# mojing1999/jmcodec

Measured on AMD Instinct MI355X. Metric: decoded frames/sec @1080p H.264 + bit-exact YUV, higher is better.
Workload: dtype u8

## Files before the change

### jmcodec_amd/csrc/decoder.cpp

```cpp
#include "decoder.h"
#include "numa.h"
#include <pthread.h>
#include <time.h>
#include "engine.h"
#include "host_copy.h"
#include "kernels.h"
#include <hip/hip_runtime_api.h>
#include <algorithm>
#include <cstdio>
#include <cstdlib>
#include <cstring>
#include <thread>

namespace jmamd {

#define HIP_OK(expr) ((expr) == hipSuccess)

namespace {
int thread_budget() {
    const char *e = getenv("JM_AMD_DEC_THREADS");
    int n = e ? atoi(e) : (int)std::thread::hardware_concurrency();
    if (!e) {
        if (FILE *f = fopen("/sys/fs/cgroup/cpu.max", "r")) {
            long long q = 0, per = 0; char qs[32] = {0};
// ... 129 lines not shown
    if (k == "field_pictures") return stat_field_pics_.load();
    if (k == "lone_fields") return stat_lone_fields_.load();
    if (k == "frames") return num_frames_;
    if (k == "out_width") return out_w_;
    if (k == "out_height") return out_h_;
    if (k == "scaled_frames") return stat_scaled_;
    if (k == "rgb_frames") return stat_rgb_;
    if (k == "deint_frames") return stat_deint_;
    if (k == "field_rate_pairs") return stat_pairs_;
    if (k == "interlaced_sequence") return codec_ == 0 && seq_active_ && !seq_.frame_mbs_only ? 1 : 0;
    if (k == "out_frame_bytes") { std::lock_guard<std::mutex> lk(const_cast<std::mutex &>(mtx_));
        return (long long)(cur_out_ ? cur_out_->fbytes : !ready_.empty() ? ready_.front()->fbytes : frame_bytes_); }
    if (k == "out_slot_bytes") { std::lock_guard<std::mutex> lk(const_cast<std::mutex &>(mtx_)); long long n = 0;
        for (const OutSlot *o : all_out_) n += (o->host ? (long long)o->bytes : 0) + (o->dev ? (long long)o->bytes : 0); return n; }
    if (k == "vui_full_range") return vui_[0];
    if (k == "vui_primaries") return vui_[1];
    if (k == "vui_transfer") return vui_[2];
    if (k == "vui_matrix") return vui_[3];
    if (k == "color_matrix") return color_matrix_;
    if (k == "color_range") return color_range_;
    if (k == "pictures") return stat_pictures_;
    if (k == "job_bytes") return stat_job_bytes_;
    if (k == "job_regrown") return stat_job_regrown_;
    if (k == "job_slot_bytes") { long long n = 0; for (auto &j : jobs_) n += (long long)j.cap; return n; }
    if (k == "errors") return stat_errors_;
    if (k == "jpeg_pictures") return stat_jpeg_pics_;
    if (k == "jpeg_sampling") return codec_ == 2 && seq_active_ ? j_sampling_ : 0;
    if (k == "jpeg_restart_intervals") return stat_jpeg_ri_;
    if (k == "copy_engines") return copier_ ? (long long)copier_->engine_mask() : 0;
    if (k == "direct_frames") return stat_direct_;
    if (k == "direct_ns") return stat_direct_ns_;
    if (k == "device_wait_errors") return stat_wait_errors_;
    if (k == "intra_mbs") return stat_intra_mbs_;
    if (k == "coef_int16") return stat_coef_;
    if (k == "syntax_digest") return codec_ == 1 ? (long long)hdigest_.h : (long long)digest_.h;
    if (k == "job_digest") return (long long)job_digest_;
    if (k == "digest_mbs") return codec_ == 1 ? (long long)hdigest_.n_cu : (long long)digest_.mbs;
    if (k == "i_pictures") return stat_i_;
    if (k == "p_pictures") return stat_p_;
    if (k == "b_pictures") return stat_b_;
    if (k == "fps_num") return codec_ == 1 ? (long long)hsps_.time_scale : (long long)seq_.time_scale;
    if (k == "fps_den") return codec_ == 1 ? (long long)hsps_.num_units_in_tick : 2ll * seq_.num_units_in_tick;
    if (k == "out_fps_num") { const bool chosen = deint_when_ == 1 || (codec_ == 0 && seq_active_ && !seq_.frame_mbs_only);
        return (field_rate() && chosen ? 2 : 1) * get_stat("fps_num"); }
    if (k == "out_fps_den") return get_stat("fps_den");
    if (k == "frames_done_unfetched") return (long long)frames_done_unfetched();
    if (k == "frames_waiting") { std::lock_guard<std::mutex> lk(const_cast<std::mutex &>(mtx_)); return (long long)ready_.size(); }
    if (k == "pictures_in_flight") { std::lock_guard<std::mutex> lk(const_cast<std::mutex &>(mtx_)); return (long long)outstanding_; }
    if (k == "coded_width") return mb_w_ * 16;
    if (k == "coded_height") return mb_h_ * 16;
    if (k == "pitch") return pitch_;
    if (k == "device") return device_;
    if (k == "threads") return pool_threads(numa_node_);
    if (k == "numa_node") return numa_node_;
    if (k == "elapsed_us") return (long long)(elapsed_ms_ * 1000.0);
    if (k == "parse_ns_i") return stat_parse_ns_i_;
    if (k == "submit_ns") return stat_submit_ns_;
    if (k == "wait_slot_ns") return stat_wait_slot_ns_;
    if (k == "parse_ns_p") return stat_parse_ns_p_;
    if (k.rfind("k_", 0) == 0 || k.rfind("eng_", 0) == 0) {
        static const char *kn[kKernelClasses] = {"inter", "intra", "deblock", "packout", "chain", "rgb_pack", "deint", "jpeg"};
        if (!engine_) return 0;
        EngineStats es = engine_->stats();
        for (int i = 0; i < kKernelClasses; i++) {
            if (k == std::string("k_") + kn[i] + "_ns") return (long long)es.ns[i];
            if (k == std::string("k_") + kn[i] + "_n") return es.launches[i];
// ... 1073 lines not shown
    mv_ext_buf.resize((size_t)n_mbs * (big_rec ? kBiRecInt16 : 32));
    const size_t fixed = (size_t)n_mbs * sizeof(MbRec) + 256 * sizeof(SliceRec);
    MbRec *mbs = nullptr; SliceRec *srec = nullptr; int16_t *coef = nullptr;
    MbRec blank; memset(&blank, 0, sizeof blank); blank.kind = MB_INTER;
    { int8_t c = -1; for (auto &s : t->slices) if (s.sh.type != SL_I && s.refs.slot[0][0] >= 0) { c = s.refs.slot[0][0]; break; }
      blank.ref[0] = blank.ref[1] = blank.ref[2] = blank.ref[3] = c; }
    JobWriter w;
    SyntaxDigest dg = digest_;
    for (int attempt = 0;; attempt++) {
        scratch.begin_picture();
        mbs = (MbRec *)js.host; srec = (SliceRec *)(js.host + (size_t)n_mbs * sizeof(MbRec)); coef = (int16_t *)(srec + 256);
        w = JobWriter();
        w.mbs = mbs; w.mv_ext = mv_ext_buf.data(); w.mv_ext_cap = (uint32_t)n_mbs * (big_rec ? kBiRecInt16 / 2 : 16);
        w.coef = coef;
        {
            long long room = (long long)js.cap - (long long)fixed - 64;
            if (room <= 0) { t->error = "job buffer too small for this picture"; stat_errors_++; fail(t->error); room = 0; }
            w.coef_cap = (uint32_t)(room / 2);
        }
        dg = digest_;
        t->n_intra = 0; t->n_i8x8 = 0; t->any_deblock = false; t->any_wp = false; t->error.clear();
        const char *first_error = nullptr; bool overflow = false;
        for (size_t si = 0; si < t->slices.size(); si++) {
            SliceTask &s = t->slices[si];
            srec[si].alpha_off = (int8_t)s.sh.alpha_off; srec[si].beta_off = (int8_t)s.sh.beta_off; srec[si].disable = (uint8_t)s.sh.disable_deblock;
            srec[si].pad = 0;
            if (s.sh.disable_deblock != 1) t->any_deblock = true;
            BitReader br(s.rbsp.data(), s.rbsp_len);
            br.set_end_from_trailing();
            br.skip_bytes(s.sh.data_bit_offset >> 3); br.skip((int)(s.sh.data_bit_offset & 7));
            if (s.sh.first_mb >= n_mbs) { t->error = "first_mb_in_slice out of range"; continue; }
            if (s.col) s.col->wait();
            if (s.has_wp) t->any_wp = true;
            SliceParseResult r = parse_slice_data(t->sps, t->pps, s.sh, br, (int)si, s.refs, scratch, w, want_digest_ ? &dg : nullptr, fast_parse_ &&
                !t->field);
            t->n_intra += r.n_intra; t->n_i8x8 += r.n_i8x8;
            if (r.error) { t->error = r.error; if (!first_error) first_error = r.error; overflow |= strcmp(r.error, "coefficient buffer overflow") == 0; }
        }
        if (overflow && js.cap < job_cap_max_ && attempt < 6 && !failed_) {
            const bool i_pic = !t->slices.empty() && t->slices[0].sh.type == SL_I;
            const size_t want = std::min(job_cap_max_, std::max(js.cap * 2, i_pic ? i_job_peak_.load() * 5 / 4 : (size_t)0));
            if (ensure_job_cap(js, want)) { stat_job_regrown_++; continue; }
        }
        if (!t->error.empty()) { stat_errors_++; note_error(std::string("slice data: ") + t->error); }
        break;
    }
    for (int i = 0; i < n_mbs; i++) if (scratch.slice_of[i] < 0) mbs[i] = blank;
    if (want_digest_) digest_ = dg;
    if (const char *dm = getenv("JM_AMD_DEC_DUMP_MB")) {
        int dp = 0, dx = 0, dy = 0;
        if (sscanf(dm, "%d:%d:%d", &dp, &dx, &dy) == 3 && (dp < 0 || dp == (int)stat_pictures_.load())) {
            for (int oy = -1; oy <= 0; oy++) for (int ox = -1; ox <= 1; ox++) {
                const int x = dx + ox, y = dy + oy;
                if (x < 0 || y < 0 || x >= t->sps.mb_w || y >= t->sps.mb_h || (oy == 0 && ox == 1)) continue;
                const MbRec &m = mbs[y * t->sps.mb_w + x];
                fprintf(stderr, "MB(%d,%d) kind %d flags 0x%02x modes 0x%02x qp %d slice %d cbp_blk 0x%04x i4 %02x%02x%02x%02x%02x%02x%02x%02x "
                        "n_intra %d n_i8x8 %d slice_type %d\n", x, y, m.kind, m.flags, m.modes, m.qp, m.slice, m.cbp_blk,
                        m.u.i4[0], m.u.i4[1], m.u.i4[2], m.u.i4[3], m.u.i4[4], m.u.i4[5], m.u.i4[6], m.u.i4[7], t->n_intra, t->n_i8x8,
                            t->slices.empty() ? -1 : (int)t->slices[0].sh.type);
            }
        }
    }
    t->n_slices = (int)t->slices.size();
    if (t->mf) {
        MotionField &f = *t->mf;
        size_t n = (size_t)n_mbs;
        f.mv[0].assign(scratch.mv.begin(), scratch.mv.begin() + n * 32); f.mv[1].assign(scratch.mv1.begin(), scratch.mv1.begin() + n * 32);
        f.ref[0].assign(scratch.refidx.begin(), scratch.refidx.begin() + n * 4); f.ref[1].assign(scratch.refidx1.begin(), scratch.refidx1.begin() + n * 4);
        f.uid[0].assign(scratch.uid0.begin(), scratch.uid0.begin() + n * 4); f.uid[1].assign(scratch.uid1.begin(), scratch.uid1.begin() + n * 4);
// ... 359 lines not shown
```

### jmcodec_amd/csrc/decoder.h

```cpp
#pragma once
#include "h264_cavlc.h"
#include "h264_syntax.h"
#include "hevc_slice.h"
#include "jpeg_syntax.h"
#include "jobs.h"
#include "scale_packed.h"
#include <atomic>
#include <chrono>
#include <condition_variable>
#include <deque>
#include <memory>
#include <mutex>
#include <string>
#include <vector>

struct ihipStream_t; struct ihipEvent_t;

namespace jmamd {

constexpr int kMaxJobSlots = 64;
constexpr int kJobSlots = 24;
constexpr int kJobSlotsSmall = 40;
constexpr int kJpegJobSlots = 16, kJpegSurfaces = 18;

// ... 224 lines not shown
    std::deque<std::unique_ptr<PicTask>> inflight_;
    std::mutex submit_mtx_;
    JobSlot jobs_[kMaxJobSlots]; int n_jobs_ = kJobSlots;
    bool n_jobs_set_ = false;
    BigJobBuf big_[kBigJobBufs];
    void free_job_buffers();
    std::deque<OutSlot *> ready_;
    std::atomic<int> done_unfetched_{0};
    std::vector<OutSlot *> free_out_, all_out_;
    OutSlot *cur_out_ = nullptr;
    int outstanding_ = 0, parse_pending_ = 0;

    struct EngineDecoderState *eng_state_ = nullptr;
    class Engine *engine_ = nullptr;
    uint8_t *surf_[kMaxSurfaces] = {nullptr};
    uint8_t *surf_block_ = nullptr;
    void free_surfaces();
    bool use_lds_deblock_ = false;
    uint8_t *resid_ = nullptr; bool use_lds_intra_ = false; bool lds_intra8_ = false;
    uint8_t *hevc_work_[kHevcWorkSets] = {nullptr, nullptr, nullptr, nullptr}; unsigned hevc_work_rr_ = 0;
    uint8_t *hevc_bs_ = nullptr; size_t hevc_bs_set_bytes_ = 0, hevc_bs_off_[4] = {0, 0, 0, 0};
    int pitch_ = 0, chroma_off_ = 0; size_t surf_bytes_ = 0, frame_bytes_ = 0, job_cap_ = 0, job_cap_max_ = 0;
    std::atomic<size_t> i_job_peak_{0};
    std::atomic<long long> stat_job_regrown_{0};
    bool gpu_open_ = false;

    bool eof_flag_ = false, is_exit_ = false;
    std::atomic<bool> eos_sent_{false};
    uint32_t num_frames_ = 0;
    std::chrono::steady_clock::time_point t0_; bool timer_started_ = false; double elapsed_ms_ = 0;
    char info_[1024];
    std::atomic<long long> stat_parse_ns_i_{0}, stat_parse_ns_p_{0}, stat_submit_ns_{0}, stat_wait_slot_ns_{0};
    std::atomic<long long> stat_pictures_{0}, stat_job_bytes_{0}, stat_errors_{0}, stat_intra_mbs_{0}, stat_coef_{0}, stat_wait_errors_{0};
    SyntaxDigest digest_;
    bool fast_parse_ = true, want_job_digest_ = false;
    std::atomic<long long> stat_direct_{0}, stat_direct_ns_{0};
    HostCopier *copier_ = nullptr; uint64_t out_sig_ = 0;
    int display_delay_ = 0;
    uint64_t job_digest_ = 1469598103934665603ull;
    HevcParamSets hps_; HevcSps hsps_; HevcPps hpps_;
    int h_poc_tid0_ = 0, h_max_dpb_ = 1, h_reorder_ = 0, extra_surf_ = 0; bool h_first_picture_ = true, h_no_rasl_output_ = false, h_seen_eos_ = false;
    HevcSliceHeader h_last_sh_; bool h_have_last_sh_ = false;
    HevcDigest hdigest_;
    long long stat_i_ = 0, stat_p_ = 0, stat_b_ = 0;
    std::vector<int> display_pocs_;
    std::vector<uint8_t> display_fields_;
    std::vector<uint32_t> display_pics_;
    uint32_t display_count_ = 0;
    JpegSplitter jsplit_; JpegTables jtab_;
    int j_w_ = 0, j_h_ = 0, j_sampling_ = 0; unsigned j_surf_rr_ = 0;
    std::atomic<long long> stat_jpeg_pics_{0}, stat_jpeg_ri_{0};
    struct TraceRec { uint64_t seq; long long t_dispatch, t_parsed, t_submit0, t_submit1; int is_i; };
    std::vector<TraceRec> trace_; bool trace_on_ = false;
};

void pool_submit(Decoder *d, PicTask *t);
int  pool_threads(int numa_node);

}
```

### jmcodec_amd/csrc/h264_cavlc.cpp

```cpp
#include "h264_cavlc.h"
#include "h264_cabac.h"
#include <mutex>
#include <stddef.h>
#include <emmintrin.h>

namespace jmamd {

static const uint8_t kTokLen[3][68] = {
{ 1,0,0,0, 6,2,0,0, 8,6,3,0, 9,8,7,5, 10,9,8,6, 11,10,9,7, 13,11,10,8, 13,13,11,9, 13,13,13,10,
 14,14,13,11, 14,14,14,13, 15,15,14,14, 15,15,15,14, 16,15,15,15, 16,16,16,15, 16,16,16,16, 16,16,16,16 },
{ 2,0,0,0, 6,2,0,0, 6,5,3,0, 7,6,6,4, 8,6,6,4, 8,7,7,5, 9,8,8,6, 11,9,9,6, 11,11,11,7,
 12,11,11,9, 12,12,12,11, 12,12,12,11, 13,13,13,12, 13,13,13,13, 13,14,13,13, 14,14,14,13, 14,14,14,14 },
{ 4,0,0,0, 6,4,0,0, 6,5,4,0, 6,5,5,4, 7,5,5,4, 7,5,5,4, 7,6,6,4, 7,6,6,4, 8,7,7,5,
 8,8,7,6, 9,8,8,7, 9,9,8,8, 9,9,9,8, 10,9,9,9, 10,10,10,10, 10,10,10,10, 10,10,10,10 } };
static const uint8_t kTokBits[3][68] = {
{ 1,0,0,0, 5,1,0,0, 7,4,1,0, 7,6,5,3, 7,6,5,3, 7,6,5,4, 15,6,5,4, 11,14,5,4, 8,10,13,4,
 15,14,9,4, 11,10,13,12, 15,14,9,12, 11,10,13,8, 15,1,9,12, 11,14,13,8, 7,10,9,12, 4,6,5,8 },
{ 3,0,0,0, 11,2,0,0, 7,7,3,0, 7,10,9,5, 7,6,5,4, 4,6,5,6, 7,6,5,8, 15,6,5,4, 11,14,13,4,
 15,10,9,4, 11,14,13,12, 8,10,9,8, 15,14,13,12, 11,10,9,12, 7,11,6,8, 9,8,10,1, 7,6,5,4 },
{ 15,0,0,0, 15,14,0,0, 11,15,13,0, 8,12,14,12, 15,10,11,11, 11,8,9,10, 9,14,13,9, 8,10,9,8, 15,14,13,13,
 11,14,10,12, 15,10,13,12, 11,14,9,12, 8,10,13,8, 13,7,9,12, 9,12,11,10, 5,8,7,6, 1,4,3,2 } };
static const uint8_t kCdcLen[20] = { 2,0,0,0, 6,1,0,0, 6,6,3,0, 6,7,7,6, 6,8,8,7 };
static const uint8_t kCdcBits[20] = { 1,0,0,0, 7,1,0,0, 4,6,1,0, 3,3,2,5, 2,3,2,0 };
static const uint8_t kTzLen[15][16] = {
// ... 91 lines not shown
    mb_w = w; mb_h = h;
    size_t n = (size_t)w * h;
    tc.assign(n * 24, 0); mv.assign(n * 32, 0); refidx.assign(n * 4, -1); i4.assign(n * 16, 2); info.assign(n, 0); slice_of.assign(n, -1);
    cbp.assign(n, 0); cmode.assign(n, 0); cbf.assign(n, 0); mvd.assign(n * 32, 0);
    mv1.assign(n * 32, 0); refidx1.assign(n * 4, -1); mvd1.assign(n * 32, 0); direct8.assign(n, 0); uid0.assign(n * 4, -1); uid1.assign(n * 4, -1);
}
void ParseScratch::begin_picture() { std::fill(slice_of.begin(), slice_of.end(), (int16_t)-1); }

namespace {

struct Canon {
    uint32_t addr; uint8_t kind , qp, cmode, i16mode; uint8_t i4[16]; int8_t ref[4];
    int16_t mv[16][2];
    int16_t i16dc[16], luma[16][16], cdc[2][4], cac[2][4][16];
    int8_t ref1[4]; int16_t mv1[16][2];
};
static_assert(sizeof(Canon) == 4 + 4 + 16 + 4 + 64 + 32 + 512 + 16 + 256 + 4 + 64, "Canon must be packed");

struct P {
    const SeqParams &sps; const PicParamSet &pps; const SliceHeader &sh;
    BitReader &br; ParseScratch &cx; JobWriter &out; SyntaxDigest *dg;
    int slice_num; const SliceRefs &rf;
    int mb_w, mb_x = 0, mb_y = 0, addr = 0, qp;
    int nA = -1, nB = -1, nC = -1, nD = -1;
    uint8_t *tc; int16_t *mv; int8_t *ref; uint8_t *i4m;
    int16_t *mvl[2]; int8_t *refl[2]; uint8_t *mvdl[2];
    uint32_t decoded_mask = 0;
    Canon *canon = nullptr;
    Cabac *cb = nullptr;
    const uint8_t *zz4 = kZigzag4, *zz8 = kZigzag8; int fld_ctx = 0;
    bool last_dqp = false;
    uint8_t *mvd = nullptr;
    const char *err = nullptr;

    void locate(int a) {
        if (a == addr + 1 && mb_x + 1 < mb_w) mb_x++; else { mb_x = a % mb_w; mb_y = a / mb_w; }
        addr = a;
        const int16_t *so = cx.slice_of.data();
        const int16_t sn = (int16_t)slice_num;
        nA = (mb_x > 0 && so[a - 1] == sn) ? a - 1 : -1;
        if (mb_y > 0) {
            const int b = a - mb_w;
            nB = so[b] == sn ? b : -1; nC = (mb_x + 1 < mb_w && so[b + 1] == sn) ? b + 1 : -1; nD = (mb_x > 0 && so[b - 1] == sn) ? b - 1 : -1;
        } else nB = nC = nD = -1;
        tc = &cx.tc[(size_t)a * 24]; mv = &cx.mv[(size_t)a * 32]; ref = &cx.refidx[(size_t)a * 4]; i4m = &cx.i4[(size_t)a * 16]; mvd = &cx.mvd[(size_t)a * 32];
        mvl[0] = mv; mvl[1] = &cx.mv1[(size_t)a * 32]; refl[0] = ref; refl[1] = &cx.refidx1[(size_t)a * 4]; mvdl[0] = mvd; mvdl[1] = &cx.mvd1[(size_t)a * 32];
    }
    __attribute__((always_inline)) inline void locate_next(int a, int first) {
        if (a == addr + 1 && mb_x + 1 < mb_w) mb_x++; else { mb_x = a % mb_w; mb_y = a / mb_w; }
        addr = a;
        const int b = a - mb_w;
        nA = (mb_x > 0 && a - 1 >= first) ? a - 1 : -1;
        nB = b >= first ? b : -1;
        nC = (mb_x + 1 < mb_w && b + 1 >= first) ? b + 1 : -1;
        nD = (mb_x > 0 && b - 1 >= first) ? b - 1 : -1;
        tc = &cx.tc[(size_t)a * 24]; mv = &cx.mv[(size_t)a * 32]; ref = &cx.refidx[(size_t)a * 4]; i4m = &cx.i4[(size_t)a * 16]; mvd = &cx.mvd[(size_t)a * 32];
        mvl[0] = mv; mvl[1] = &cx.mv1[(size_t)a * 32]; refl[0] = ref; refl[1] = &cx.refidx1[(size_t)a * 4]; mvdl[0] = mvd; mvdl[1] = &cx.mvd1[(size_t)a * 32];
    }
    bool intra_usable(int n) const { return n >= 0 && (!pps.constrained_intra || (cx.info[n] & 1)); }

    int nc_luma(int bx, int by) const {
        int a = -1, b = -1;
        if (bx > 0) a = tc[by * 4 + bx - 1]; else if (nA >= 0) a = cx.tc[(size_t)nA * 24 + by * 4 + 3];
        if (by > 0) b = tc[(by - 1) * 4 + bx]; else if (nB >= 0) b = cx.tc[(size_t)nB * 24 + 12 + bx];
        if (a >= 0 && b >= 0) return (a + b + 1) >> 1;
        return a >= 0 ? a : (b >= 0 ? b : 0);
    }
    int nc_chroma(int pl, int bx, int by) const {
        int o = 16 + 4 * pl, a = -1, b = -1;
        if (bx > 0) a = tc[o + by * 2]; else if (nA >= 0) a = cx.tc[(size_t)nA * 24 + o + by * 2 + 1];
        if (by > 0) b = tc[o + bx]; else if (nB >= 0) b = cx.tc[(size_t)nB * 24 + o + 2 + bx];
        if (a >= 0 && b >= 0) return (a + b + 1) >> 1;
        return a >= 0 ? a : (b >= 0 ? b : 0);
    }

    __attribute__((always_inline)) inline int residual_block(int nCtx, int max_num, int first, int16_t *dst, const uint8_t *map) {
        uint32_t e;
        if (nCtx < 0) { e = g_cdc[br.peek(8)]; }
        else if (nCtx >= 8) { e = g_tok_flc[br.peek(6)]; }
        else {
            const TokTable &T = g_tok[nCtx < 2 ? 0 : (nCtx < 4 ? 1 : 2)];
            uint32_t v = br.peek(16);
            e = T.t[v >> 8];
            if ((e & 0xff) == 0xff) e = T.t[256 * (e >> 8) + (v & 0xff)];
        }
        int len = e & 0xff;
        if (len == 0) return -1;
        br.skip(len);
        int total = (int)(e >> 10), t1 = (e >> 8) & 3;
        if (total == 0) return 0;
        if (total > max_num) return -1;
        return residual_levels(total, t1, max_num, first, dst, map);
    }
    __attribute__((noinline)) int residual_levels(int total, int t1, int max_num, int first, int16_t *dst, const uint8_t *map) {
        return levels_of(br, total, t1, max_num, first, dst, map); }
    __attribute__((always_inline)) static inline int levels_of(BitReader &br, int total, int t1, int max_num, int first, int16_t *dst, const uint8_t *map) {
        memset(dst, 0, max_num == 4 ? 8 : 32);
        if (total == 1 && t1 == 1) {
            const int v = 1 - 2 * (int)br.u1();
            int z;
            if (max_num == 4) { const uint8_t e = g_ctz[0][br.peek(3)]; if (!(e & 15)) return -1; br.skip(e & 15); z = e >> 4; }
            else { const uint16_t e = g_tz[0][br.peek(9)]; if (!(e & 0xff)) return -1; br.skip(e & 0xff); z = e >> 8; }
            if (z + 1 > max_num) return -1;
            dst[map[z + first]] = (int16_t)v;
            return 1;
        }
        int level[16];
        int suffix_len = (total > 10 && t1 < 3) ? 1 : 0;
        int i = 0;
        {
            const uint32_t s3 = br.peek(3);
            level[0] = 1 - (int)((s3 >> 1) & 2); level[1] = 1 - (int)(s3 & 2); level[2] = 1 - (int)((s3 << 1) & 2);
            br.skip(t1); i = t1;
        }
        for (; i < total; i++) {
            uint32_t w = br.peek(32);
            if (w == 0) return -1;
            int prefix = __builtin_clz(w);
            int code;
            if (prefix < 14) {
                code = (prefix << suffix_len) + (int)((w >> (31 - prefix - suffix_len)) & ((1u << suffix_len) - 1));
                br.skip(prefix + 1 + suffix_len);
            } else {
                br.skip(prefix + 1);
                code = (prefix < 15 ? prefix : 15) << suffix_len;
                int size = (prefix == 14 && suffix_len == 0) ? 4 : (prefix >= 15 ? prefix - 3 : suffix_len);
                if (size > 0) code += (int)br.u(size);
                if (prefix >= 15 && suffix_len == 0) code += 15;
                if (prefix >= 16) code += (1 << (prefix - 3)) - 4096;
            }
            if (i == t1 && t1 < 3) code += 2;
            int lv = (code & 1) ? (-code - 1) >> 1 : (code + 2) >> 1;
            level[i] = lv;
            if (suffix_len == 0) suffix_len = 1;
            int a = lv < 0 ? -lv : lv;
            if (a > (3 << (suffix_len - 1)) && suffix_len < 6) suffix_len++;
        }
        int zeros_left = 0;
        if (total < max_num) {
            if (max_num == 4) { uint8_t z = g_ctz[total - 1][br.peek(3)]; if (!(z & 15)) return -1; br.skip(z & 15); zeros_left = z >> 4; }
            else { uint16_t z = g_tz[total - 1][br.peek(9)]; if (!(z & 0xff)) return -1; br.skip(z & 0xff); zeros_left = z >> 8; }
            if (zeros_left + total > max_num) return -1;
        }
        int pos = zeros_left + total - 1;
        for (i = 0; i < total; i++) {
            dst[map[pos + first]] = (int16_t)level[i];
            if (i == total - 1) break;
            int run = 0;
            if (zeros_left > 0) {
                if (zeros_left <= 6) { uint8_t r = g_run[zeros_left - 1][br.peek(3)]; br.skip(r & 15); run = r >> 4; }
                else {
                    uint32_t w3 = br.peek(3);
                    if (w3) { run = 7 - (int)w3; br.skip(3); }
                    else { uint32_t w = br.peek(16); if (!w) return -1; int lz = __builtin_clz(w) - 16; run = lz + 4; br.skip(lz + 1); }
                }
                if (run > zeros_left) return -1;
// ... 211 lines not shown
        cx.direct8[addr] |= (uint8_t)mask;
        return true;
    }
    void mark8(int q) { int bx = (q & 1) * 2, by = (q >> 1) * 2;
        decoded_mask |= (1u << (by * 4 + bx)) | (1u << (by * 4 + bx + 1)) | (1u << (by * 4 + bx + 4)) | (1u << (by * 4 + bx + 5)); }

    bool skip_mb() {
        MbRec *r = begin_mb();
        r->kind = MB_INTER; r->qp = (uint8_t)qp;
        cx.info[addr] = 4; last_dqp = false;
        if (sh.type == SL_B) {
            cx.direct8[addr] = 16;
            if (!direct_pred(15)) return false;
            write_motion(r, true);
            finish_mb(r);
            return err == nullptr;
        }
        int px = 0, py = 0;
        if (nA >= 0 && nB >= 0) {
            Nb A = nb(-1, 0), B = nb(0, -1);
            if (!((A.ref == 0 && !A.mvx && !A.mvy) || (B.ref == 0 && !B.mvx && !B.mvy))) predict(0, 0, 4, 0, 0, 0, px, py);
        }
        ref[0] = ref[1] = ref[2] = ref[3] = 0;
        set_mv(0, 0, 4, 4, px, py);
        write_motion(r, false);
        finish_mb(r);
        return err == nullptr;
    }


    struct Nv { int ref, x, y; };
    inline Nv nbv(int m, int r, int b8) const {
        if (m < 0) return Nv{-2, 0, 0};
        const int16_t *q = &cx.mv[(size_t)m * 32 + r * 2];
        return Nv{cx.refidx[(size_t)m * 4 + b8], q[0], q[1]};
    }
    inline void mvp16(int refi, const Nv &A, const Nv &B, int &px, int &py) const {
        const Nv C = nC >= 0 ? nbv(nC, 12, 2) : nbv(nD, 15, 3);
        if (B.ref == -2 && C.ref == -2 && A.ref != -2) { px = A.x; py = A.y; return; }
        const int ma = A.ref == refi, mb = B.ref == refi, mc = C.ref == refi;
        if (ma + mb + mc == 1) { const Nv &n = ma ? A : (mb ? B : C); px = n.x; py = n.y; }
        else { px = med(A.x, B.x, C.x); py = med(A.y, B.y, C.y); }
    }
    inline void put_inter16(MbRec *r, int refi, int x, int y, uint32_t coef_off, uint32_t flags, uint32_t cbp_blk, uint32_t cbp_cac) {
        const uint32_t v = (uint32_t)(uint16_t)x | ((uint32_t)(uint16_t)y << 16);
        const uint64_t vv = (uint64_t)v << 32 | v;
        uint64_t *d = (uint64_t *)mv;
        for (int i = 0; i < 8; i++) d[i] = vv;
        const uint32_t rr = (uint8_t)refi * 0x01010101u;
        memcpy(ref, &rr, 4);
        cx.slice_of[addr] = (int16_t)slice_num;
        if (rf.track_uid) {
            int32_t *u0 = &cx.uid0[(size_t)addr * 4], *u1 = &cx.uid1[(size_t)addr * 4];
            const int32_t u = rf.uid[0][refi];
            u0[0] = u0[1] = u0[2] = u0[3] = u; u1[0] = u1[1] = u1[2] = u1[3] = -1;
            refl[1][0] = refl[1][1] = refl[1][2] = refl[1][3] = -1;
            cx.direct8[addr] = 0;
        }
        const int my = (int16_t)y, mx = (int16_t)x;
        if (my > out.max_mvy) out.max_mvy = my;
        if (mx > out.max_mvx) out.max_mvx = mx;
        static_assert(MB_INTER == 0 && offsetof(MbRec, cbp_blk) == 4 && offsetof(MbRec, coef_off) == 8 && offsetof(MbRec, ref) == 12 && offsetof(MbRec,
            u) == 16, "record layout");
        uint64_t *q = (uint64_t *)r;
        q[0] = (uint64_t)(uint8_t)qp << 8 | (uint64_t)(flags | MBF_DECODED) << 24 | (uint64_t)cbp_blk << 32 | (uint64_t)cbp_cac << 48 |
            (uint64_t)(uint8_t)slice_num << 56;
        q[1] = (uint64_t)coef_off | (uint64_t)((uint8_t)rf.slot[0][refi] * 0x01010101u) << 32;
        q[2] = vv; q[3] = vv;
    }
    __attribute__((always_inline)) inline void skip_mb_fast() {
        int px = 0, py = 0;
        if (nA >= 0 && nB >= 0) {
            const Nv A = nbv(nA, 3, 1), B = nbv(nB, 12, 2);
            if (!((A.ref == 0 && !A.x && !A.y) || (B.ref == 0 && !B.x && !B.y))) mvp16(0, A, B, px, py);
        }
        memset(tc, 0, 24);
        cx.info[addr] = 4;
        put_inter16(&out.mbs[addr], 0, px, py, out.coef_count, 0, 0, 0);
    }
    static inline int nc_of(int s) { return s < 64 ? (s + 1) >> 1 : s & 31; }
    __attribute__((always_inline)) static inline int token_fast(BitReader &br, int sum) {
        const int cls = kTokClassOfSum.t[sum];
        const uint32_t v = br.peek(16);
        if (cls == 0 && (v & 0x8000)) { br.skip(1); return 0; }
        const TokTable &T = g_tok[cls];
        uint32_t e = T.t[v >> 8];
        if ((e & 0xff) == 0xff) e = T.t[256 * (e >> 8) + (v & 0xff)];
        const int len = e & 0xff;
        if (len == 0) return -1;
        br.skip(len);
        return (int)(e >> 8);
    }
    __attribute__((always_inline)) inline bool residual_fast(BitReader &br, int cbp, const bool i16, uint32_t &flags, uint32_t &bits, uint32_t &cbm) {
        static const uint8_t ident[16] = {0,1,2,3,4,5,6,7,8,9,10,11,12,13,14,15};
        static const uint8_t kWin[16] = {9, 10, 17, 18, 11, 12, 19, 20, 25, 26, 33, 34, 27, 28, 35, 36};
        static const uint8_t kRas[16] = {0, 1, 4, 5, 2, 3, 6, 7, 8, 9, 12, 13, 10, 11, 14, 15};
        alignas(8) uint8_t w[5 * 8];
        const uint8_t *ta = nA >= 0 ? &cx.tc[(size_t)nA * 24] : nullptr, *tb = nB >= 0 ? &cx.tc[(size_t)nB * 24] : nullptr;
        flags = bits = cbm = 0;
        memset(tc, 0, 24);
        const uint32_t need = (i16 ? 16u : 0u) + 64u * (uint32_t)__builtin_popcount(cbp & 15) + ((cbp & 0x30) ? 8u : 0u) + ((cbp & 0x20) ? 128u : 0u);
        if (out.coef_count + need > out.coef_cap) { err = "coefficient buffer overflow"; return false; }
        if ((cbp & 15) || i16) {
            memset(w, 0, sizeof w);
            if (tb) memcpy(w + 1, tb + 12, 4); else memset(w + 1, 64, 4);
            for (int j = 0; j < 4; j++) w[8 * (j + 1)] = ta ? ta[4 * j + 3] : 64;
            if (i16) {
                int16_t *d = alloc_coef(16); if (!d) return false;
                const int tk = token_fast(br, w[8] + w[1]);
                if (tk < 0 || (tk && levels_of(br, tk >> 2, tk & 3, 16, 0, d, zz4) < 0)) { err = "entropy error (Intra16x16 DC)"; return false; }
            }
            const int max_num = i16 ? 15 : 16, first = i16 ? 1 : 0;
            for (int b8 = 0; b8 < 4; b8++) {
                if (!(cbp & (1 << b8))) continue;
                for (int k = 0; k < 4; k++) {
                    const int blk = b8 * 4 + k, wi = kWin[blk];
                    const int tk = token_fast(br, w[wi - 1] + w[wi - 8]);
                    if (tk < 0) { err = "entropy error (luma block)"; return false; }
                    if (!tk) continue;
                    const int total = tk >> 2;
                    int16_t *d = out.coef + out.coef_count;
                    if (total > max_num || levels_of(br, total, tk & 3, max_num, first, d, zz4) < 0) { err = "entropy error (luma block)"; return false; }
                    w[wi] = (uint8_t)total; tc[kRas[blk]] = (uint8_t)total; bits |= 1u << blk; out.coef_count += 16;
                }
            }
        }
        if (cbp & 0x30) {
            for (int pl = 0; pl < 2; pl++) {
                int16_t *d = out.coef + out.coef_count;
                const uint32_t e = g_cdc[br.peek(8)];
                if (!(e & 0xff)) { err = "entropy error (chroma DC)"; return false; }
                br.skip((int)(e & 0xff));
                if (!(e >> 10)) continue;
                if ((int)(e >> 10) > 4 || levels_of(br, (int)(e >> 10), (int)(e >> 8) & 3, 4, 0, d, ident) < 0) { err = "entropy error (chroma DC)";
                    return false; }
                flags |= pl ? MBF_CR_DC : MBF_CB_DC; out.coef_count += 4;
            }
        }
        if (cbp & 0x20) {
            for (int pl = 0; pl < 2; pl++) {
                const int o = 16 + 4 * pl;
                uint8_t c[9];
                c[1] = tb ? tb[o + 2] : 64; c[2] = tb ? tb[o + 3] : 64; c[3] = ta ? ta[o + 1] : 64; c[6] = ta ? ta[o + 3] : 64;
                for (int k = 0; k < 4; k++) {
                    const int ci = 4 + (k >> 1) * 3 + (k & 1);
                    const int tk = token_fast(br, c[ci - 1] + c[ci - 3]);
                    if (tk < 0 || (tk >> 2) > 15) { err = "entropy error (chroma AC)"; return false; }
                    c[ci] = (uint8_t)(tk >> 2);
                    if (!tk) continue;
                    int16_t *d = out.coef + out.coef_count;
                    if (levels_of(br, tk >> 2, tk & 3, 15, 1, d, zz4) < 0) { err = "entropy error (chroma AC)"; return false; }
                    tc[o + k] = (uint8_t)(tk >> 2); cbm |= 1u << (4 * pl + k); out.coef_count += 16;
                }
            }
        }
        return true;
    }
    __attribute__((always_inline)) inline bool p16x16_fast(BitReader &br) {
        int refi = 0;
        const int nref = sh.num_ref_idx[0];
        if (nref > 1) { refi = br.te(nref - 1); if (refi >= nref) { err = "ref_idx out of range"; return false; } }
        int px, py;
        mvp16(refi, nbv(nA, 3, 1), nbv(nB, 12, 2), px, py);
        const int dx = br.se(), dy = br.se();
        const uint32_t code = br.ue();
        if (code > 47) { err = "bad coded_block_pattern"; return false; }
        const int cbp = kCbpInter[code];
        MbRec *r = &out.mbs[addr];
        cx.info[addr] = 0;
        if (cbp) {
            const int dqp = br.se();
            if (dqp < -26 || dqp > 25) { err = "mb_qp_delta out of range"; return false; }
            qp += dqp; if (qp < 0) qp += 52; else if (qp > 51) qp -= 52;
            const uint32_t coef_off = out.coef_count;
            uint32_t flags, bits, cbm;
            if (!residual_fast(br, cbp, false, flags, bits, cbm)) return false;
            put_inter16(r, refi, px + dx, py + dy, coef_off, flags, bits, cbm);
        } else {
            memset(tc, 0, 24);
            put_inter16(r, refi, px + dx, py + dy, out.coef_count, 0, 0, 0);
        }
        if (br.overrun()) { err = "macroblock data truncated"; return false; }
        return true;
    }

    inline void skip_mb_fast_ae() {
        skip_mb_fast();
        cx.cbp[addr] = 0; cx.cmode[addr] = 0; cx.cbf[addr] = 0; memset(mvd, 0, 32); last_dqp = false;
    }
    bool p16x16_fast_ae() {
        MbRec *r = &out.mbs[addr];
        cx.info[addr] = 0; cx.cbp[addr] = 0; cx.cmode[addr] = 0; cx.cbf[addr] = 0;
        memset(tc, 0, 24);
        int refi = 0;
        const int nref = sh.num_ref_idx[0];
        if (nref > 1) { refi = ae_ref_idx(0, 0, 0); if (err || refi >= nref) { if (!err) err = "ref_idx out of range"; return false; } }
        int px, py, dx, dy;
        mvp16(refi, nbv(nA, 3, 1), nbv(nB, 12, 2), px, py);
        read_mvd(0, 0, 4, 4, dx, dy, 0);
        if (err) return false;
        const int cbp = ae_cbp();
        cx.cbp[addr] = (uint8_t)cbp;
        bool t8 = false;
        if ((cbp & 15) && pps.transform8x8) { t8 = ae_t8x8() != 0; if (t8) cx.info[addr] |= 8; }
        if (cbp) {
            const int dqp = ae_qp_delta();
            if (err || dqp < -26 || dqp > 25) { if (!err) err = "mb_qp_delta out of range"; return false; }
            qp += dqp; if (qp < 0) qp += 52; else if (qp > 51) qp -= 52;
            last_dqp = dqp != 0;
        } else last_dqp = false;
        put_inter16(r, refi, px + dx, py + dy, out.coef_count, 0, 0, 0);
        if (t8) r->modes |= MBM_T8X8;
        if (cbp && !residual(r, cbp, false, t8, false)) return false;
        if (cb->overrun) { err = "macroblock data truncated"; return false; }
        return true;
// ... 421 lines not shown
                        if (rf_[l][i] < 0) { mark8(i); continue; }
                        int nsp = st == 0 ? 1 : (st == 3 ? 4 : 2), bw = (st == 0 || st == 1) ? 2 : 1, bh = (st == 0 || st == 2) ? 2 : 1;
                        for (int p = 0; p < nsp; p++) {
                            int bx = ox + (st == 1 ? 0 : (st == 2 ? p : (p & 1))), by = oy + (st == 1 ? p : (st == 2 ? 0 : (p >> 1)));
                            int px, py, dx, dy; predict(bx, by, bw, rf_[l][i], 0, 0, px, py, l);
                            read_mvd(bx, by, bw, bh, dx, dy, l);
                            set_mv(bx, by, bw, bh, px + dx, py + dy, l);
                        }
                    }
                }
            }
            if (err) return false;
            write_motion(r, sub8);
            if (err) return false;
            if (!i16) {
                if (cb) cbp = ae_cbp();
                else { uint32_t code = br.ue(); if (code > 47) { err = "bad coded_block_pattern"; return false; } cbp = kCbpInter[code]; }
                if ((cbp & 15) && pps.transform8x8 && !sub8) { t8 = cb ? ae_t8x8() : br.u1(); if (t8) cx.info[addr] |= 8; }
            }
        }
        if (itype >= 0 && !i16) {
            if (cb) cbp = ae_cbp();
            else { uint32_t code = br.ue(); if (code > 47) { err = "bad coded_block_pattern"; return false; } cbp = kCbpIntra[code]; }
        }
        if (cb) cx.cbp[addr] = (uint8_t)cbp;
        if (t8) r->modes |= MBM_T8X8;
        if (cbp > 0 || i16) {
            int dqp = cb ? ae_qp_delta() : br.se();
            if (dqp < -26 || dqp > 25) { err = "mb_qp_delta out of range"; return false; }
            qp = (qp + dqp + 52) % 52;
            last_dqp = dqp != 0;
        } else last_dqp = false;
        r->qp = (uint8_t)qp;
        if ((cbp > 0 || i16) && !cb && !t8 && !canon) {
            BitReader b = br;
            uint32_t fl, bits, cbm;
            const bool ok = i16 ? residual_fast(b, cbp, true, fl, bits, cbm) : residual_fast(b, cbp, false, fl, bits, cbm);
            br = b;
            if (!ok) return false;
            r->flags |= (uint8_t)fl; r->cbp_blk = (uint16_t)bits; r->cbp_cac = (uint8_t)cbm;
        } else if (cbp > 0 || i16) { if (!residual(r, cbp, i16, t8, itype >= 0)) return false; }
        if (err) return false;
        if (cb ? cb->overrun : br.overrun()) { err = "macroblock data truncated"; return false; }
        if (canon && t8) r->kind |= 16;
        finish_mb(r);
        r->kind &= 15;
        return true;
    }
};

}

SliceParseResult parse_slice_data(const SeqParams &sps, const PicParamSet &pps, const SliceHeader &sh,
                                  BitReader &br, int slice_num, const SliceRefs &refs,
                                  ParseScratch &cx, JobWriter &out, SyntaxDigest *digest, bool allow_fast) {
    cavlc_init_tables();
    SliceParseResult res;
    Canon canon;
    P p{sps, pps, sh, br, cx, out, digest, slice_num, refs, sps.mb_w};
    p.qp = sh.qp;
    p.canon = digest ? &canon : nullptr;
    if (sh.field_pic) { p.zz4 = kFieldScan.s4; p.zz8 = kFieldScan.s8; p.fld_ctx = 277 - 105; allow_fast = false; }
    int n_mbs = sps.mb_w * sps.mb_h, addr = sh.first_mb;
    if (pps.cabac) {
        static thread_local Cabac cabac;
        while (!br.aligned()) if (!br.u1()) { res.error = "cabac_alignment_one_bit is not 1"; return res; }
        if (sh.cabac_init_idc > 2) { res.error = "bad cabac_init_idc"; return res; }
        cabac.init_contexts(sh.type == SL_I ? 0 : 1 + sh.cabac_init_idc, sh.qp);
        cabac.init_engine(br.byte_ptr(), br.base() + br.size());
        p.cb = &cabac;
        const bool fast_ae = allow_fast && sh.type == SL_P && !digest && !refs.bipred_rec;
        for (;;) {
            if (addr >= n_mbs) { res.error = "slice runs past the end of the picture"; return res; }
            bool ok;
            if (fast_ae) {
                p.locate_next(addr, sh.first_mb);
                if (p.ae_mb_skip()) { p.skip_mb_fast_ae(); ok = true; }
                else {
                    const int mb_type = p.ae_mb_type();
                    ok = mb_type == 0 ? p.p16x16_fast_ae() : p.macroblock(res.n_intra, res.n_i8x8, mb_type);
                }
            } else {
                p.locate(addr);
                if (sh.type != SL_I && p.ae_mb_skip()) ok = p.skip_mb();
                else ok = p.macroblock(res.n_intra, res.n_i8x8);
            }
            if (!ok) { res.error = p.err ? p.err : "macroblock error"; return res; }
            addr++; res.mbs_decoded++;
            if (cabac.overrun || cabac.bits_consumed() > (size_t)(cabac.end - cabac.start) * 8 + 16) { res.error = "slice data truncated"; return res; }
            if (cabac.terminate()) break;
        }
        return res;
    }
    if (allow_fast && sh.type == SL_P && !digest && !pps.transform8x8 && !refs.bipred_rec) {
        BitReader b = br;
        bool more = true;
        while (more) {
            const uint32_t run = b.ue();
            if (b.overrun() || run > (uint32_t)(n_mbs - addr)) { res.error = "bad mb_skip_run"; break; }
            for (uint32_t i = 0; i < run; i++) { p.locate_next(addr, sh.first_mb); p.skip_mb_fast(); addr++; }
            res.mbs_decoded += (int)run;
            if (run > 0) more = b.more_rbsp_data();
            if (!more) break;
            if (addr >= n_mbs) { res.error = "slice runs past the end of the picture"; break; }
            p.locate_next(addr, sh.first_mb);
            const uint32_t mb_type = b.ue();
            bool ok;
            if (mb_type == 0) ok = p.p16x16_fast(b);
            else { br = b; ok = p.macroblock(res.n_intra, res.n_i8x8, (int)(mb_type > 255 ? 255 : mb_type)); b = br; }
            if (!ok) { res.error = p.err ? p.err : "macroblock error"; break; }
            addr++; res.mbs_decoded++;
            more = b.more_rbsp_data();
        }
        br = b;
        return res;
    }
    bool more = true;
    while (more) {
        if (sh.type != SL_I) {
            uint32_t run = br.ue();
            if (br.overrun() || run > (uint32_t)(n_mbs - addr)) { res.error = "bad mb_skip_run"; return res; }
            for (uint32_t i = 0; i < run; i++) { p.locate(addr); if (!p.skip_mb()) { res.error = p.err; return res; } addr++; res.mbs_decoded++; }
            if (run > 0) more = br.more_rbsp_data();
            if (!more) break;
        }
        if (addr >= n_mbs) { res.error = "slice runs past the end of the picture"; return res; }
        p.locate(addr);
        if (!p.macroblock(res.n_intra, res.n_i8x8)) { res.error = p.err ? p.err : "macroblock error"; return res; }
        addr++; res.mbs_decoded++;
        more = br.more_rbsp_data();
    }
    return res;
}

}
```

### jmcodec_amd/csrc/h264_cavlc.h

```cpp
#pragma once
#include "h264_syntax.h"
#include "jobs.h"
#include <condition_variable>
#include <mutex>
#include <vector>

namespace jmamd {

struct JobWriter {
    MbRec   *mbs = nullptr;
    int16_t *mv_ext = nullptr;  uint32_t mv_ext_count = 0, mv_ext_cap = 0;
    int16_t *coef = nullptr;    uint32_t coef_count = 0, coef_cap = 0;
    int max_mvx = 0;
    int max_mvy = 0;
};

struct ParseScratch {
    int mb_w = 0, mb_h = 0;
    std::vector<uint8_t> tc;
    std::vector<int16_t> mv;
    std::vector<int8_t>  refidx;
    std::vector<uint8_t> i4;
    std::vector<uint8_t> info;
    std::vector<int16_t> slice_of;
// ... 2 lines not shown
    void resize(int w, int h);
    void begin_picture();
};

struct MotionField {
    std::vector<int16_t> mv[2];
    std::vector<int8_t>  ref[2];
    std::vector<int32_t> uid[2];
    std::vector<uint8_t> intra;
    std::mutex m; std::condition_variable cv; bool done = false;
    void wait() { std::unique_lock<std::mutex> lk(m); cv.wait(lk, [&] { return done; }); }
    void publish() { { std::lock_guard<std::mutex> lk(m); done = true; } cv.notify_all(); }
};

struct SliceRefs {
    int8_t  slot[2][32];
    int32_t uid[2][32];
    int32_t poc[2][32];
    uint8_t is_long[2][32];
    int32_t cur_poc = 0;
    const MotionField *col = nullptr;
    int col_mode = 0, cur_parity = 0;
    bool track_uid = false;
    bool bipred_rec = false;
};

struct SyntaxDigest { uint64_t h = 1469598103934665603ull; uint64_t mbs = 0; };

struct SliceParseResult {
    int mbs_decoded = 0;
    int n_intra = 0;
    int n_i8x8 = 0;
    const char *error = nullptr;
};

SliceParseResult parse_slice_data(const SeqParams &sps, const PicParamSet &pps, const SliceHeader &sh,
                                  BitReader &br, int slice_num, const SliceRefs &refs,
                                  ParseScratch &cx, JobWriter &out, SyntaxDigest *digest, bool allow_fast = true);

void cavlc_init_tables();

}
```

Measured before the change: 15170.

## Add fast CAVLC intra macroblock path and split neighbour pointer setup

```diff
diff --git a/jmcodec_amd/csrc/decoder.cpp b/jmcodec_amd/csrc/decoder.cpp
--- a/jmcodec_amd/csrc/decoder.cpp
+++ b/jmcodec_amd/csrc/decoder.cpp
@@ -185,6 +185,10 @@
     if (k == "direct_ns") return stat_direct_ns_;
     if (k == "device_wait_errors") return stat_wait_errors_;
     if (k == "intra_mbs") return stat_intra_mbs_;
+    {
+        static const char *fk[5] = {"fast_skip_mbs", "fast_p16_mbs", "fast_i4_mbs", "fast_i16_mbs", "level_escapes"};
+        for (int i = 0; i < 5; i++) if (k == fk[i]) return stat_fast_[i];
+    }
     if (k == "coef_int16") return stat_coef_;
     if (k == "syntax_digest") return codec_ == 1 ? (long long)hdigest_.h : (long long)digest_.h;
     if (k == "job_digest") return (long long)job_digest_;
@@ -1324,9 +1328,10 @@
             if (s.sh.first_mb >= n_mbs) { t->error = "first_mb_in_slice out of range"; continue; }
             if (s.col) s.col->wait();
             if (s.has_wp) t->any_wp = true;
-            SliceParseResult r = parse_slice_data(t->sps, t->pps, s.sh, br, (int)si, s.refs, scratch, w, want_digest_ ? &dg : nullptr, fast_parse_ &&
-                !t->field);
+            SliceParseResult r = parse_slice_data(t->sps, t->pps, s.sh, br, (int)si, s.refs, scratch, w, want_digest_ ? &dg : nullptr, fast_parse_);
             t->n_intra += r.n_intra; t->n_i8x8 += r.n_i8x8;
+            {   const int f[5] = {r.fast_skip, r.fast_p16, r.fast_i4, r.fast_i16, r.level_escapes};
+                for (int i = 0; i < 5; i++) if (f[i]) stat_fast_[i] += f[i]; }
             if (r.error) { t->error = r.error; if (!first_error) first_error = r.error; overflow |= strcmp(r.error, "coefficient buffer overflow") == 0; }
         }
         if (overflow && js.cap < job_cap_max_ && attempt < 6 && !failed_) {
diff --git a/jmcodec_amd/csrc/decoder.h b/jmcodec_amd/csrc/decoder.h
--- a/jmcodec_amd/csrc/decoder.h
+++ b/jmcodec_amd/csrc/decoder.h
@@ -280,6 +280,7 @@
     char info_[1024];
     std::atomic<long long> stat_parse_ns_i_{0}, stat_parse_ns_p_{0}, stat_submit_ns_{0}, stat_wait_slot_ns_{0};
     std::atomic<long long> stat_pictures_{0}, stat_job_bytes_{0}, stat_errors_{0}, stat_intra_mbs_{0}, stat_coef_{0}, stat_wait_errors_{0};
+    std::atomic<long long> stat_fast_[5] = {};
     SyntaxDigest digest_;
     bool fast_parse_ = true, want_job_digest_ = false;
     std::atomic<long long> stat_direct_{0}, stat_direct_ns_{0};
diff --git a/jmcodec_amd/csrc/h264_cavlc.cpp b/jmcodec_amd/csrc/h264_cavlc.cpp
--- a/jmcodec_amd/csrc/h264_cavlc.cpp
+++ b/jmcodec_amd/csrc/h264_cavlc.cpp
@@ -147,6 +147,9 @@
     bool last_dqp = false;
     uint8_t *mvd = nullptr;
     const char *err = nullptr;
+    SliceParseResult *st = nullptr;
+    uint8_t *tc0 = nullptr; int16_t *mv0 = nullptr; int8_t *ref0 = nullptr;
+    bool fast_resid = true;
 
     void locate(int a) {
         if (a == addr + 1 && mb_x + 1 < mb_w) mb_x++; else { mb_x = a % mb_w; mb_y = a / mb_w; }
@@ -169,8 +172,12 @@
         nB = b >= first ? b : -1;
         nC = (mb_x + 1 < mb_w && b + 1 >= first) ? b + 1 : -1;
         nD = (mb_x > 0 && b - 1 >= first) ? b - 1 : -1;
-        tc = &cx.tc[(size_t)a * 24]; mv = &cx.mv[(size_t)a * 32]; ref = &cx.refidx[(size_t)a * 4]; i4m = &cx.i4[(size_t)a * 16]; mvd = &cx.mvd[(size_t)a * 32];
-        mvl[0] = mv; mvl[1] = &cx.mv1[(size_t)a * 32]; refl[0] = ref; refl[1] = &cx.refidx1[(size_t)a * 4]; mvdl[0] = mvd; mvdl[1] = &cx.mvd1[(size_t)a * 32];
+        tc = tc0 + (size_t)a * 24; mv = mv0 + (size_t)a * 32; ref = ref0 + (size_t)a * 4;
+    }
+    inline void locate_rest() {
+        const size_t a = (size_t)addr;
+        i4m = &cx.i4[a * 16]; mvd = &cx.mvd[a * 32];
+        mvl[0] = mv; mvl[1] = &cx.mv1[a * 32]; refl[0] = ref; refl[1] = &cx.refidx1[a * 4]; mvdl[0] = mvd; mvdl[1] = &cx.mvd1[a * 32];
     }
     bool intra_usable(int n) const { return n >= 0 && (!pps.constrained_intra || (cx.info[n] & 1)); }
 
@@ -208,8 +215,9 @@
         return residual_levels(total, t1, max_num, first, dst, map);
     }
     __attribute__((noinline)) int residual_levels(int total, int t1, int max_num, int first, int16_t *dst, const uint8_t *map) {
-        return levels_of(br, total, t1, max_num, first, dst, map); }
-    __attribute__((always_inline)) static inline int levels_of(BitReader &br, int total, int t1, int max_num, int first, int16_t *dst, const uint8_t *map) {
+        return levels_of(br, total, t1, max_num, first, dst, map, st->level_escapes); }
+    __attribute__((always_inline)) static inline int levels_of(BitReader &br, int total, int t1, int max_num, int first, int16_t *dst, const uint8_t *map,
+                                                               int &escapes) {
         memset(dst, 0, max_num == 4 ? 8 : 32);
         if (total == 1 && t1 == 1) {
             const int v = 1 - 2 * (int)br.u1();
@@ -237,6 +245,7 @@
                 code = (prefix << suffix_len) + (int)((w >> (31 - prefix - suffix_len)) & ((1u << suffix_len) - 1));
                 br.skip(prefix + 1 + suffix_len);
             } else {
+                escapes++;
                 br.skip(prefix + 1);
                 code = (prefix < 15 ? prefix : 15) << suffix_len;
                 int size = (prefix == 14 && suffix_len == 0) ? 4 : (prefix >= 15 ? prefix - 3 : suffix_len);
@@ -514,8 +523,8 @@
     struct Nv { int ref, x, y; };
     inline Nv nbv(int m, int r, int b8) const {
         if (m < 0) return Nv{-2, 0, 0};
-        const int16_t *q = &cx.mv[(size_t)m * 32 + r * 2];
-        return Nv{cx.refidx[(size_t)m * 4 + b8], q[0], q[1]};
+        const int16_t *q = mv0 + (size_t)m * 32 + r * 2;
+        return Nv{ref0[(size_t)m * 4 + b8], q[0], q[1]};
     }
     inline void mvp16(int refi, const Nv &A, const Nv &B, int &px, int &py) const {
         const Nv C = nC >= 0 ? nbv(nC, 12, 2) : nbv(nD, 15, 3);
@@ -536,7 +545,7 @@
             int32_t *u0 = &cx.uid0[(size_t)addr * 4], *u1 = &cx.uid1[(size_t)addr * 4];
             const int32_t u = rf.uid[0][refi];
             u0[0] = u0[1] = u0[2] = u0[3] = u; u1[0] = u1[1] = u1[2] = u1[3] = -1;
-            refl[1][0] = refl[1][1] = refl[1][2] = refl[1][3] = -1;
+            memset(&cx.refidx1[(size_t)addr * 4], -1, 4);
             cx.direct8[addr] = 0;
         }
         const int my = (int16_t)y, mx = (int16_t)x;
@@ -578,7 +587,7 @@
         static const uint8_t kWin[16] = {9, 10, 17, 18, 11, 12, 19, 20, 25, 26, 33, 34, 27, 28, 35, 36};
         static const uint8_t kRas[16] = {0, 1, 4, 5, 2, 3, 6, 7, 8, 9, 12, 13, 10, 11, 14, 15};
         alignas(8) uint8_t w[5 * 8];
-        const uint8_t *ta = nA >= 0 ? &cx.tc[(size_t)nA * 24] : nullptr, *tb = nB >= 0 ? &cx.tc[(size_t)nB * 24] : nullptr;
+        const uint8_t *ta = nA >= 0 ? tc0 + (size_t)nA * 24 : nullptr, *tb = nB >= 0 ? tc0 + (size_t)nB * 24 : nullptr;
         flags = bits = cbm = 0;
         memset(tc, 0, 24);
         const uint32_t need = (i16 ? 16u : 0u) + 64u * (uint32_t)__builtin_popcount(cbp & 15) + ((cbp & 0x30) ? 8u : 0u) + ((cbp & 0x20) ? 128u : 0u);
@@ -590,11 +599,12 @@
             if (i16) {
                 int16_t *d = alloc_coef(16); if (!d) return false;
                 const int tk = token_fast(br, w[8] + w[1]);
-                if (tk < 0 || (tk && levels_of(br, tk >> 2, tk & 3, 16, 0, d, zz4) < 0)) { err = "entropy error (Intra16x16 DC)"; return false; }
+                if (tk < 0 || (tk && levels_of(br, tk >> 2, tk & 3, 16, 0, d, zz4, st->level_escapes) < 0)) { err = "entropy error (Intra16x16 DC)";
+                    return false; }
             }
             const int max_num = i16 ? 15 : 16, first = i16 ? 1 : 0;
-            for (int b8 = 0; b8 < 4; b8++) {
-                if (!(cbp & (1 << b8))) continue;
+            for (uint32_t left = cbp & 15; left; left &= left - 1) {
+                const int b8 = __builtin_ctz(left);
                 for (int k = 0; k < 4; k++) {
                     const int blk = b8 * 4 + k, wi = kWin[blk];
                     const int tk = token_fast(br, w[wi - 1] + w[wi - 8]);
@@ -602,7 +612,8 @@
                     if (!tk) continue;
                     const int total = tk >> 2;
                     int16_t *d = out.coef + out.coef_count;
-                    if (total > max_num || levels_of(br, total, tk & 3, max_num, first, d, zz4) < 0) { err = "entropy error (luma block)"; return false; }
+                    if (total > max_num || levels_of(br, total, tk & 3, max_num, first, d, zz4, st->level_escapes) < 0) { err = "entropy error (luma block)";
+                        return false; }
                     w[wi] = (uint8_t)total; tc[kRas[blk]] = (uint8_t)total; bits |= 1u << blk; out.coef_count += 16;
                 }
             }
@@ -614,8 +625,8 @@
                 if (!(e & 0xff)) { err = "entropy error (chroma DC)"; return false; }
                 br.skip((int)(e & 0xff));
                 if (!(e >> 10)) continue;
-                if ((int)(e >> 10) > 4 || levels_of(br, (int)(e >> 10), (int)(e >> 8) & 3, 4, 0, d, ident) < 0) { err = "entropy error (chroma DC)";
-                    return false; }
+                if ((int)(e >> 10) > 4 || levels_of(br, (int)(e >> 10), (int)(e >> 8) & 3, 4, 0, d, ident, st->level_escapes) < 0) {
+                    err = "entropy error (chroma DC)"; return false; }
                 flags |= pl ? MBF_CR_DC : MBF_CB_DC; out.coef_count += 4;
             }
         }
@@ -631,7 +642,7 @@
                     c[ci] = (uint8_t)(tk >> 2);
                     if (!tk) continue;
                     int16_t *d = out.coef + out.coef_count;
-                    if (levels_of(br, tk >> 2, tk & 3, 15, 1, d, zz4) < 0) { err = "entropy error (chroma AC)"; return false; }
+                    if (levels_of(br, tk >> 2, tk & 3, 15, 1, d, zz4, st->level_escapes) < 0) { err = "entropy error (chroma AC)"; return false; }
                     tc[o + k] = (uint8_t)(tk >> 2); cbm |= 1u << (4 * pl + k); out.coef_count += 16;
                 }
             }
@@ -663,6 +674,75 @@
             put_inter16(r, refi, px + dx, py + dy, out.coef_count, 0, 0, 0);
         }
         if (br.overrun()) { err = "macroblock data truncated"; return false; }
+        return true;
+    }
+
+    __attribute__((noinline)) bool intra_fast(int itype) {
+        BitReader b = br;
+        const bool ok = intra_fast_on(b, itype);
+        br = b;
+        return ok;
+    }
+    __attribute__((always_inline)) inline bool intra_fast_on(BitReader &br, int itype) {
+        const bool i16 = itype != 0;
+        uint64_t modes64 = 0;
+        uint32_t modes = 0;
+        int cbp;
+        if (!i16) {
+            alignas(8) int8_t m[5 * 8];
+            if (nB >= 0) { if (cx.info[nB] & 2) memcpy(m + 1, &cx.i4[(size_t)nB * 16 + 12], 4); else memset(m + 1, 2, 4); } else memset(m + 1, -1, 4);
+            if (nA >= 0) { const uint8_t *l = &cx.i4[(size_t)nA * 16]; const bool nxn = (cx.info[nA] & 2) != 0;
+                for (int j = 0; j < 4; j++) m[8 * (j + 1)] = nxn ? (int8_t)l[4 * j + 3] : (int8_t)2; }
+            else for (int j = 0; j < 4; j++) m[8 * (j + 1)] = -1;
+            static const uint8_t kWin[16] = {9, 10, 17, 18, 11, 12, 19, 20, 25, 26, 33, 34, 27, 28, 35, 36};
+            for (int blk = 0; blk < 16; blk++) {
+                const int wi = kWin[blk];
+                int pred = m[wi - 1] < m[wi - 8] ? m[wi - 1] : m[wi - 8];
+                if (pred < 0) pred = 2;
+                const uint32_t v = br.peek(4);
+                const int rem = (int)(v & 7), mode = (v & 8) ? pred : rem + (rem >= pred);
+                br.skip((v & 8) ? 1 : 4);
+                m[wi] = (int8_t)mode;
+            }
+            for (int j = 0; j < 4; j++) {
+                uint32_t row; memcpy(&row, m + 8 * (j + 1) + 1, 4); memcpy(i4m + 4 * j, &row, 4);
+                modes64 |= (uint64_t)((row & 15) | (row >> 4 & 0xf0) | (row >> 8 & 0xf00) | (row >> 12 & 0xf000)) << (16 * j);
+            }
+            const uint32_t cm = br.ue();
+            if (cm > 3) return false;
+            modes = cm;
+            const uint32_t code = br.ue();
+            if (code > 47) return false;
+            cbp = kCbpIntra[code];
+        } else {
+            const int k = itype - 1;
+            cbp = (((k >> 2) % 3) << 4) | (k >= 12 ? 15 : 0);
+            const uint32_t cm = br.ue();
+            if (cm > 3) return false;
+            modes = (uint32_t)((k & 3) << 2) | cm;
+        }
+        const uint32_t coef_off = out.coef_count;
+        uint32_t flags = 0, bits = 0, cbm = 0;
+        if (cbp > 0 || i16) {
+            const int dqp = br.se();
+            if (dqp < -26 || dqp > 25) return false;
+            qp += dqp; if (qp < 0) qp += 52; else if (qp > 51) qp -= 52;
+            if (!residual_fast(br, cbp, i16, flags, bits, cbm)) return false;
+        } else memset(tc, 0, 24);
+        if (br.overrun()) return false;
+        flags |= (uint32_t)MBF_DECODED | (nA >= 0 ? MBF_AVAIL_A : 0) | (nB >= 0 ? MBF_AVAIL_B : 0) | (nC >= 0 ? MBF_AVAIL_C : 0) | (nD >= 0 ? MBF_AVAIL_D : 0);
+        cx.info[addr] = i16 ? 1 : 3;
+        cx.slice_of[addr] = (int16_t)slice_num;
+        memset(ref, -1, 4); memset(mv, 0, 64);
+        if (rf.track_uid) { memset(refl[1], -1, 4); memset(mvl[1], 0, 64); memset(mvdl[1], 0, 32); cx.direct8[addr] = 0; }
+        static_assert(offsetof(MbRec, modes) == 2 && offsetof(MbRec, flags) == 3 && offsetof(MbRec, cbp_cac) == 6 && offsetof(MbRec, slice) == 7,
+            "record layout");
+        uint64_t *q = (uint64_t *)&out.mbs[addr];
+        q[0] = (uint64_t)(i16 ? MB_I16 : MB_I4) | (uint64_t)(uint8_t)qp << 8 | (uint64_t)modes << 16 | (uint64_t)flags << 24 | (uint64_t)bits << 32 |
+            (uint64_t)cbm << 48 | (uint64_t)(uint8_t)slice_num << 56;
+        q[1] = (uint64_t)coef_off | 0xffffffffull << 32;
+        q[2] = modes64; q[3] = 0;
+        if (i16) st->fast_i16++; else st->fast_i4++;
         return true;
     }
 
@@ -1150,7 +1230,7 @@
             last_dqp = dqp != 0;
         } else last_dqp = false;
         r->qp = (uint8_t)qp;
-        if ((cbp > 0 || i16) && !cb && !t8 && !canon) {
+        if ((cbp > 0 || i16) && !cb && !t8 && !canon && fast_resid) {
             BitReader b = br;
             uint32_t fl, bits, cbm;
             const bool ok = i16 ? residual_fast(b, cbp, true, fl, bits, cbm) : residual_fast(b, cbp, false, fl, bits, cbm);
@@ -1178,6 +1258,8 @@
     P p{sps, pps, sh, br, cx, out, digest, slice_num, refs, sps.mb_w};
     p.qp = sh.qp;
     p.canon = digest ? &canon : nullptr;
+    p.st = &res; p.fast_resid = allow_fast;
+    p.tc0 = cx.tc.data(); p.mv0 = cx.mv.data(); p.ref0 = cx.refidx.data();
     if (sh.field_pic) { p.zz4 = kFieldScan.s4; p.zz8 = kFieldScan.s8; p.fld_ctx = 277 - 105; allow_fast = false; }
     int n_mbs = sps.mb_w * sps.mb_h, addr = sh.first_mb;
     if (pps.cabac) {
@@ -1192,7 +1274,7 @@
             if (addr >= n_mbs) { res.error = "slice runs past the end of the picture"; return res; }
             bool ok;
             if (fast_ae) {
-                p.locate_next(addr, sh.first_mb);
+                p.locate_next(addr, sh.first_mb); p.locate_rest();
                 if (p.ae_mb_skip()) { p.skip_mb_fast_ae(); ok = true; }
                 else {
                     const int mb_type = p.ae_mb_type();
@@ -1217,15 +1299,45 @@
             const uint32_t run = b.ue();
             if (b.overrun() || run > (uint32_t)(n_mbs - addr)) { res.error = "bad mb_skip_run"; break; }
             for (uint32_t i = 0; i < run; i++) { p.locate_next(addr, sh.first_mb); p.skip_mb_fast(); addr++; }
-            res.mbs_decoded += (int)run;
+            res.mbs_decoded += (int)run; res.fast_skip += (int)run;
             if (run > 0) more = b.more_rbsp_data();
             if (!more) break;
             if (addr >= n_mbs) { res.error = "slice runs past the end of the picture"; break; }
             p.locate_next(addr, sh.first_mb);
             const uint32_t mb_type = b.ue();
             bool ok;
-            if (mb_type == 0) ok = p.p16x16_fast(b);
-            else { br = b; ok = p.macroblock(res.n_intra, res.n_i8x8, (int)(mb_type > 255 ? 255 : mb_type)); b = br; }
+            if (mb_type == 0) { ok = p.p16x16_fast(b); res.fast_p16++; }
+            else {
+                ok = false;
+                p.locate_rest();
+                if (mb_type - 5 < 25 && !pps.constrained_intra) {
+                    const BitReader b0 = b; const int qp0 = p.qp; const uint32_t cc0 = out.coef_count;
+                    br = b; ok = p.intra_fast((int)mb_type - 5); b = br;
+                    if (ok) res.n_intra++; else { b = b0; p.qp = qp0; out.coef_count = cc0; p.err = nullptr; }
+                }
+                if (!ok) { br = b; ok = p.macroblock(res.n_intra, res.n_i8x8, (int)(mb_type > 255 ? 255 : mb_type)); b = br; }
+            }
+            if (!ok) { res.error = p.err ? p.err : "macroblock error"; break; }
+            addr++; res.mbs_decoded++;
+            more = b.more_rbsp_data();
+        }
+        br = b;
+        return res;
+    }
+    if (allow_fast && sh.type == SL_I && !digest && !pps.transform8x8) {
+        BitReader b = br;
+        bool more = true;
+        while (more) {
+            if (addr >= n_mbs) { res.error = "slice runs past the end of the picture"; break; }
+            p.locate_next(addr, sh.first_mb); p.locate_rest();
+            const uint32_t mb_type = b.ue();
+            bool ok = false;
+            if (mb_type < 25) {
+                const BitReader b0 = b; const int qp0 = p.qp; const uint32_t cc0 = out.coef_count;
+                br = b; ok = p.intra_fast((int)mb_type); b = br;
+                if (ok) res.n_intra++; else { b = b0; p.qp = qp0; out.coef_count = cc0; p.err = nullptr; }
+            }
+            if (!ok) { br = b; ok = p.macroblock(res.n_intra, res.n_i8x8, (int)(mb_type > 255 ? 255 : mb_type)); b = br; }
             if (!ok) { res.error = p.err ? p.err : "macroblock error"; break; }
             addr++; res.mbs_decoded++;
             more = b.more_rbsp_data();
diff --git a/jmcodec_amd/csrc/h264_cavlc.h b/jmcodec_amd/csrc/h264_cavlc.h
--- a/jmcodec_amd/csrc/h264_cavlc.h
+++ b/jmcodec_amd/csrc/h264_cavlc.h
@@ -58,6 +58,8 @@
     int n_intra = 0;
     int n_i8x8 = 0;
     const char *error = nullptr;
+    int fast_skip = 0, fast_p16 = 0, fast_i4 = 0, fast_i16 = 0;
+    int level_escapes = 0;
 };
 
 SliceParseResult parse_slice_data(const SeqParams &sps, const PicParamSet &pps, const SliceHeader &sh,
```

Result: slower. 12840 (-15.3%).
